# Renmusxd/IsingMonteCarlo

Hardware: AMD Instinct MI355X
Metric: spin-op updates/sec (whole node), 32×32 TFIM, 1024 replicas at 1/2/4/8 GPUs (higher is better)
Workload: dtype u32 op words, f64 acceptance arithmetic

## Files before the change

isingmontecarlo_amd/csrc/sse_cluster.hip.h:

```cpp
#pragma once
#include "sse_cluster_pass.hip.h"

namespace sse {

#define SSE_CLW 16
#define SSE_CL_MAX_VARS 4095u
#define SSE_CLE_TWO (1u << 28)
#define SSE_CLE_LONG (1u << 29)
#define SSE_CLE_CUT (1u << 31)
#define SSE_CL_TOUCHED (1u << 24)

typedef __attribute__((address_space(3))) uint32_t sse_lds_u32;
typedef __attribute__((address_space(3))) uint16_t sse_lds_u16;
typedef __attribute__((address_space(3))) uint8_t sse_lds_u8;
#define LDS32B(a) (*(sse_lds_u32 *)(uintptr_t)(a))
#define LDS16B(a) (*(sse_lds_u16 *)(uintptr_t)(a))
#define LDS8B(a) (*(sse_lds_u8 *)(uintptr_t)(a))
__device__ __forceinline__ void lds_cas32(uint32_t addr, uint32_t expect, uint32_t val) {
    (void)__hip_atomic_compare_exchange_strong((sse_lds_u32 *)(uintptr_t)addr, &expect, val, __ATOMIC_RELAXED, __ATOMIC_RELAXED, __HIP_MEMORY_SCOPE_WORKGROUP);
}

__device__ __forceinline__ uint32_t lds_ld16(uint32_t addr) {
    uint32_t v = LDS16B(addr);
    asm("" : "+v"(v));
    return v;
}
#define SSE_CL_MISC_DUMMY 12u

struct ClLds {
    uint32_t o_tab;
    uint32_t o_state;
    uint32_t o_touch;
    uint32_t o_misc;
    uint32_t o_chn;
    uint32_t o_chtr;
    uint32_t o_ent;
    uint32_t o_frozen, o_froot;
    uint32_t o_parent;
    uint32_t end;
    __host__ __device__ __forceinline__ void carve(uint32_t N, uint32_t nwords, uint32_t Nb, uint32_t ufcap, bool has_long) {
        uint32_t base = 0;
        o_tab = base; base += Nb + 1u;
        o_state = base; base += nwords;
        o_touch = base; base += nwords;
        o_misc = base; base += 16u;
        o_chn = base; base += SSE_MAX_CHUNKS;
        o_chtr = base; base += SSE_MAX_CHUNKS;
        o_ent = base; base += (uint32_t)SSE_CLW * (N + 1u);
        o_frozen = base; base += has_long ? (ufcap + 31u) / 32u : 0u;
        o_froot = base; base += has_long ? (ufcap + 31u) / 32u : 0u;
        o_parent = base;
        end = base + (ufcap + 1u) / 2u;
    }
};
static inline __host__ __device__ bool cl_ids_fit(uint32_t N, uint32_t S, uint32_t ufcap) {
    return S < ufcap && S < 65535u && ((size_t)S + 31) / 32 <= (size_t)SSE_CLW * (N + 1);
}
static inline __host__ __device__ uint32_t cl_list_cap(uint32_t N, uint32_t S) {
    const size_t tab = (size_t)SSE_CLW * (N + 1), bits = ((size_t)S + 31) / 32;
    return bits < tab ? (uint32_t)(2 * (tab - bits)) : 0u;
}

extern "C" __device__ int sse_cl_llvm_writelane(int, int, int) __asm("llvm.amdgcn.writelane.i32");
__device__ __forceinline__ uint32_t cl_writelane(uint32_t v, uint32_t x, int l) { return (uint32_t)sse_cl_llvm_writelane((int)x, l, (int)v); }

__device__ __forceinline__ uint32_t cl_union_wave(const UFA<false> &uf, uint32_t a, uint32_t b) {
    for (;;) {
        uint32_t xa = a, xb = b, pa = uf.get(a), pb = uf.get(b);
        while ((pa != xa) | (pb != xb)) { xa = pa; xb = pb; pa = uf.get(xa); pb = uf.get(xb); }
        if (a != xa) uf.set(a, xa);
        if (b != xb) uf.set(b, xb);
        if (xa == xb) return xa;
        const uint32_t lo = min(xa, xb), hi = max(xa, xb);
        uf.set(hi, lo);
        SSE_WAVE_FENCE();
        if (uf.get(hi) == lo) return lo;
        a = xa; b = xb;
    }
}

#ifndef SSE_CL_FIND_LEVELS
#define SSE_CL_FIND_LEVELS 4
#endif
template <int K, bool HAS_LONG, int PHASE>
__global__ __launch_bounds__(SSE_CLW * 64, 4) void cluster_kernel(DevBatch B, SweepArgs A) {
    constexpr int W = SSE_CLW, NT = W * 64;
    constexpr uint32_t TS = 64u * K;
    static_assert(K == 2 || K == 4, "ids are stored two rows per dword");
    ClLds L;
    L.carve(B.N, B.nwords, B.Nb, B.lds_ufcap, HAS_LONG);
    const int tid = threadIdx.x, lane = tid & 63, wave = __builtin_amdgcn_readfirstlane(tid >> 6);
    const uint32_t r = blockIdx.x;
    const uint32_t N = B.N, nwords = B.nwords;
    const int n = (int)B.n[r];
    const uint32_t C = B.ntrans[r], M = B.cutoff[r], err = B.err[r];
    if (err) return;
    const uint32_t S = N + C + (uint32_t)(W - 1) * N;
    if (n == 0 || C == 0u || !cl_ids_fit(N, S, B.lds_ufcap)) {
        if (tid == 0) B.aux[r] = 1u;
        return;
    }
    UFA<false> uf;
    uf.gparent = nullptr; uf.gfrozen = nullptr; uf.gfroot = nullptr;
    uf.o_parent = L.o_parent; uf.o_frozen = L.o_frozen; uf.o_froot = L.o_froot;
    uint64_t epoch = B.epoch[r];
    uint32_t *ops = B.ops + (size_t)r * B.stride;
    uint32_t *ids = B.segs + (size_t)r * B.stride;
    const bool DEFER = A.defer_flips != 0u && B.flipb != nullptr;
// ... 169 lines not shown
    SSE_STAMP(1);

    for (uint32_t v = tid; v < N; v += NT) {
        uint32_t t = 0;
#pragma unroll 4
        for (uint32_t w2 = 0; w2 < (uint32_t)W; ++w2) {
            const uint32_t x = LDSW(L.o_ent, w2 * (N + 1u) + v);
            t |= x;
            const uint32_t seg_end = x & 0xFFFFu;
            const uint32_t nxt = (w2 + 1u == (uint32_t)W) ? v : N + C + w2 * N + v;
            if (seg_end != nxt) uf_union(uf, seg_end, nxt);
        }
        if (t >> 24) atomicOr(&LDSW(L.o_touch, v >> 5), 1u << (v & 31));
    }
    __syncthreads();
    SSE_STAMP(2);
    const uint32_t o_bits = L.o_ent, o_list = L.o_ent + (S + 31u) / 32u;
    const uint32_t list_cap = cl_list_cap(N, S);
    uint32_t myclusters = 0;
    for (uint32_t i0 = 0; i0 < S; i0 += NT) {
        const uint32_t i = i0 + tid;
        const bool inr = i < S;
        bool isroot = false;
        if (inr) {
            const uint32_t root = uf_find_ro(uf, i);
            uf.set(i, root);
            if constexpr (HAS_LONG)
                if ((uf.frozen_get(i >> 5) >> (i & 31)) & 1u) { uf.froot_or(root >> 5, 1u << (root & 31)); LDSW(L.o_misc, MISC_ANYFROZEN) = 1u; }
            isroot = root == i;
            if (isroot & (i < N + C)) {
                const bool touched = (i >= N) || ((LDSW(L.o_touch, i >> 5) >> (i & 31)) & 1u);
                if (touched) myclusters++;
            }
        }
        const uint64_t m = sse_ballot(isroot);
        if (m) {
            uint32_t base = 0;
            if (lane == 0) base = atomicAdd(&LDSW(L.o_misc, MISC_LOOP_A), (uint32_t)popc64(m));
            base = (uint32_t)__builtin_amdgcn_readfirstlane((int)base);
            const uint32_t pos = base + popc64(m & lanemask_lt(lane));
            if (isroot && pos < list_cap) LDSH(o_list, pos) = (uint16_t)i;
        }
    }
    for (uint32_t i = tid; i < (S + 31u) / 32u; i += NT) LDSW(o_bits, i) = 0u;
    __syncthreads();
    SSE_STAMP(3);
    const Rng rng = make_rng(B, r, epoch);
    const uint32_t nroots = LDSW(L.o_misc, MISC_LOOP_A);
    if (nroots <= list_cap) {
        for (uint32_t k = tid; k < nroots; k += NT) {
            const uint32_t root = LDSH(o_list, k);
            const uint4 o = rng.draw(SSE_TAG_CLUSTER, root);
            const uint32_t isfrozen = HAS_LONG ? (uf.froot_get(root >> 5) >> (root & 31)) & 1u : 0u;
            if (!isfrozen && u01(o.x) < A.prob) atomicOr(&LDSW(o_bits, root >> 5), 1u << (root & 31));
        }
        __syncthreads();
        for (uint32_t i = tid; i < S; i += NT) {
            const uint32_t root = uf.get(i);
            uf.set(i, (LDSW(o_bits, root >> 5) >> (root & 31)) & 1u);
        }
    } else {
        for (uint32_t i = tid; i < S; i += NT) {
            const uint32_t root = uf.get(i);
            const uint4 o = rng.draw(SSE_TAG_CLUSTER, root);
            const uint32_t isfrozen = HAS_LONG ? (uf.froot_get(root >> 5) >> (root & 31)) & 1u : 0u;
            uf.set(i, (!isfrozen && u01(o.x) < A.prob) ? 1u : 0u);
        }
    }
    if (tid == 0) uf.set(S, 0u);
    {
        uint32_t c = myclusters;
        for (int off = 32; off > 0; off >>= 1) c += __shfl_down(c, off);
        if (lane == 0 && c) atomicAdd(&LDSW(L.o_misc, MISC_NCLUST), c);
    }
    __syncthreads();
    SSE_STAMP(4);

    if (DEFER) {
        uint32_t cutnext = N + cutbase;
        uint8_t *fb = B.flipb + (size_t)r * B.stride;
        constexpr int D = 3;
        const uint32_t *mskw = reinterpret_cast<const uint32_t *>(msk);
        uint32_t qid[D][K / 2], qmk[D], bpend[K];
        auto issue = [&](int slot, uint32_t pt) {
            const uint32_t pc = pt < pend ? pt : pbeg;
#pragma unroll
            for (int j = 0; j < K; j += 2) qid[slot][j / 2] = row_ld(ids, (pc >> 1) + (uint32_t)(j * 32 + lane));
            qmk[slot] = row_ld(mskw, (pc >> 6) * 4u + (uint32_t)(lane & 15));
        };
#pragma unroll
        for (int d = 0; d < D; ++d) issue(d, pbeg + (uint32_t)d * TS);
#pragma unroll
        for (int j = 0; j < K; ++j) bpend[j] = 0u;
        uint32_t pprev = pbeg;
        bool first = true;
        for (uint32_t p0 = pbeg; p0 < pend; p0 += TS) {
            uint32_t id2[K / 2];
#pragma unroll
            for (int j = 0; j < K / 2; ++j) id2[j] = qid[0][j];
            const uint32_t mkv = qmk[0];
#pragma unroll
            for (int d = 0; d + 1 < D; ++d) {
#pragma unroll
                for (int j = 0; j < K / 2; ++j) qid[d][j] = qid[d + 1][j];
                qmk[d] = qmk[d + 1];
            }
            if (!first) {
#pragma unroll
                for (int j = 0; j < K; ++j) fb[pprev + (uint32_t)(j * 64 + lane)] = (uint8_t)bpend[j];
            }
            first = false;
            pprev = p0;
            issue(D - 1, p0 + (uint32_t)D * TS);
#pragma unroll
            for (int j = 0; j < K; ++j) {
                const uint64_t cutm = (uint64_t)(uint32_t)__builtin_amdgcn_readlane((int)mkv, 4 * j) | ((uint64_t)(uint32_t)__builtin_amdgcn_readlane((int)mkv, 4 * j + 1) << 32);
                const uint32_t own = __builtin_amdgcn_mbcnt_hi((uint32_t)(cutm >> 32), __builtin_amdgcn_mbcnt_lo((uint32_t)cutm, cutnext));
                const uint32_t idin = (j & 1) ? (id2[j / 2] >> 16) : (id2[j / 2] & 0xFFFFu);
                const uint32_t f1 = LDS16B(par_b + 2u * idin), f2 = LDS16B(par_b + 2u * own);
                uint32_t m_other = (0u - f1) & 0xFu;
                if constexpr (HAS_LONG) {
                    const uint64_t twom = (uint64_t)(uint32_t)__builtin_amdgcn_readlane((int)mkv, 4 * j + 2) | ((uint64_t)(uint32_t)__builtin_amdgcn_readlane((int)mkv, 4 * j + 3) << 32);
                    m_other &= sel64(twom, vgpr_copy_u32(0xFu), vgpr_copy_u32(0x5u));
                }
                bpend[j] = sel64(cutm, f1 | (f2 << 2), m_other);
                cutnext += (uint32_t)popc64(cutm);
            }
        }
        if (pbeg < pend) {
#pragma unroll
            for (int j = 0; j < K; ++j) fb[pprev + (uint32_t)(j * 64 + lane)] = (uint8_t)bpend[j];
        }
    } else
    {
        uint32_t cutnext = N + cutbase;
        const uint32_t E1 = B.E + 1u;
        uint32_t wnext[K], inext[K / 2], wpend[K];
#pragma unroll
        for (int j = 0; j < K; ++j) { wnext[j] = row_ld(ops, pbeg + (uint32_t)(j * 64 + lane)); wpend[j] = wnext[j]; }
#pragma unroll
        for (int j = 0; j < K; j += 2) inext[j / 2] = row_ld(ids, (pbeg >> 1) + (uint32_t)(j * 32 + lane));
        uint32_t pprev = pbeg;
        for (uint32_t p0 = pbeg; p0 < pend; p0 += TS) {
            uint32_t word[K], id2[K / 2];
#pragma unroll
            for (int j = 0; j < K; ++j) word[j] = wnext[j];
#pragma unroll
            for (int j = 0; j < K / 2; ++j) id2[j] = inext[j];
            {
#pragma unroll
                for (int j = 0; j < K; ++j) row_st(ops, pprev + (uint32_t)(j * 64 + lane), wpend[j]);
                pprev = p0;
                const uint32_t pn0 = p0 + TS < pend ? p0 + TS : p0;
#pragma unroll
                for (int j = 0; j < K; ++j) wnext[j] = row_ld(ops, pn0 + (uint32_t)(j * 64 + lane));
#pragma unroll
                for (int j = 0; j < K; j += 2) inext[j / 2] = row_ld(ids, (pn0 >> 1) + (uint32_t)(j * 32 + lane));
            }
            uint32_t f1[K], f2[K];
            uint64_t cutm[K];
#pragma unroll
            for (int j = 0; j < K; ++j) {
                cutm[j] = sse_ballot(((word[j] >> 4) - E1) < N);
                const uint32_t own = __builtin_amdgcn_mbcnt_hi((uint32_t)(cutm[j] >> 32), __builtin_amdgcn_mbcnt_lo((uint32_t)cutm[j], cutnext));
                const uint32_t idin = (j & 1) ? (id2[j / 2] >> 16) : (id2[j / 2] & 0xFFFFu);
                f1[j] = LDS16B(par_b + 2u * idin);
                f2[j] = LDS16B(par_b + 2u * own);
                cutnext += (uint32_t)popc64(cutm[j]);
            }
#pragma unroll
            for (int j = 0; j < K; ++j) {
                const uint32_t allbits = (((word[j] >> 4) - 1u) < B.E) ? 0xFu : 0x5u;
                const uint32_t m_other = (0u - f1[j]) & allbits;
                const uint32_t m_cut = f1[j] | (f2[j] << 2);
                wpend[j] = word[j] ^ sel64(cutm[j], m_cut, m_other);
            }
        }
        if (pbeg < pend) {
#pragma unroll
            for (int j = 0; j < K; ++j) row_st(ops, pprev + (uint32_t)(j * 64 + lane), wpend[j]);
        }
    }
    for (uint32_t v0 = (uint32_t)wave * 64u; v0 < N; v0 += NT) {
        const uint32_t v = v0 + (uint32_t)lane;
        const uint64_t fm = sse_ballot(v < N && (uf.get(v) & 1u) != 0u);
        const uint32_t i = (v0 >> 5) + (uint32_t)lane;
        if (lane < 2 && i < nwords) LDSW(L.o_state, i) ^= (lane ? (uint32_t)(fm >> 32) : (uint32_t)fm) & LDSW(L.o_touch, i);
    }
    __syncthreads();
    SSE_STAMP(5);
    const uint32_t nclusters = LDSW(L.o_misc, MISC_NCLUST);
    epoch++;
    uint64_t a0 = 0, a1 = 0, a2 = 0, a3 = 0, a6 = 0;
    if (A.domask & SSE_DO_FREE) {
        const Rng rngf = make_rng(B, r, epoch);
        for (uint32_t v0 = (uint32_t)wave * 64u; v0 < N; v0 += NT) {
            const uint32_t v = v0 + (uint32_t)lane;
            const bool isfree = v < N && !((LDSW(L.o_touch, v >> 5) >> (v & 31u)) & 1u);
            uint32_t bit = 0u;
            if (isfree) bit = rngf.draw(SSE_TAG_FREE, v).x >> 31;
            const uint64_t fm = sse_ballot(isfree), bm = sse_ballot(bit != 0u);
            const uint32_t i = (v0 >> 5) + (uint32_t)lane;
            if (fm != 0ull && lane < 2 && i < nwords) {
                const uint32_t f = lane ? (uint32_t)(fm >> 32) : (uint32_t)fm, b = lane ? (uint32_t)(bm >> 32) : (uint32_t)bm;
                LDSW(L.o_state, i) = (LDSW(L.o_state, i) & ~f) | b;
            }
        }
        __syncthreads();
        epoch++;
    }
    if (A.sampling_freq && (A.step0 + 1) % A.sampling_freq == 0) {
        if (tid == 0) LDSW(L.o_misc, MISC_LOOP_A) = 0u;
        __syncthreads();
        uint32_t up = 0;
// ... 19 lines not shown
```

isingmontecarlo_amd/csrc/sse_core.hip.h:

```cpp
#pragma once
#include <hip/hip_runtime.h>
#include <stdint.h>
#include "../../include/sse_format.h"
#include "sse_batch.h"

namespace sse {

#ifdef SSE_PHASE_TIMING
#define SSE_STAMP(slot) do { if (threadIdx.x == 0) { const unsigned long long t_ = __builtin_amdgcn_s_memrealtime(); B.dbg[(size_t)r * 16 + (slot)] += t_ - dbg_t0; dbg_t0 = t_; } } while (0)
#define SSE_STAMP_INIT unsigned long long dbg_t0 = __builtin_amdgcn_s_memrealtime()
#else
#define SSE_STAMP(slot) do { } while (0)
#define SSE_STAMP_INIT do { } while (0)
#endif

__device__ __forceinline__ uint32_t philox_bump(uint32_t k, uint32_t w) {
    uint32_t r;
    const uint32_t ks = (uint32_t)__builtin_amdgcn_readfirstlane((int)k);
    asm volatile("s_add_u32 %0, %1, %2" : "=s"(r) : "s"(ks), "s"(w) : "scc");
    return r;
}
__device__ __forceinline__ uint4 philox4x32_10(uint32_t c0, uint32_t c1, uint32_t c2, uint32_t c3, uint32_t k0,
                                               uint32_t k1) {
#pragma unroll
    for (int i = 0; i < 10; ++i) {
        const uint64_t p0 = (uint64_t)0xD2511F53u * (uint64_t)c0, p1 = (uint64_t)0xCD9E8D57u * (uint64_t)c2;
        const uint32_t hi0 = (uint32_t)(p0 >> 32), lo0 = (uint32_t)p0, hi1 = (uint32_t)(p1 >> 32), lo1 = (uint32_t)p1;
        uint32_t n0 = __builtin_amdgcn_bitop3_b32(hi1, c1, k0, 0x96), n2 = __builtin_amdgcn_bitop3_b32(hi0, c3, k1, 0x96);
        c0 = n0; c1 = lo1; c2 = n2; c3 = lo0;
        if (i < 9) { k0 = philox_bump(k0, 0x9E3779B9u); k1 = philox_bump(k1, 0xBB67AE85u); }
    }
    return make_uint4(c0, c1, c2, c3);
}

struct Rng {
    uint32_t k0, k1, replica, epoch_lo, epoch_hi24;
#ifdef SSE_PHASE_TIMING
    uint32_t dbgx;
#endif
    __device__ __forceinline__ uint4 draw(uint32_t tag, uint32_t index) const {
#ifdef SSE_PHASE_TIMING
        if (dbgx & 2u) {
            const uint32_t h = (index * 0x9E3779B9u) ^ (epoch_lo * 0x85EBCA6Bu) ^ (replica * 0xC2B2AE35u) ^ tag;
            return make_uint4(h * 0x27D4EB2Fu, h ^ (h >> 15), h * 0x165667B1u, h ^ (h << 13));
        }
#endif
        return philox4x32_10(index, epoch_lo, replica, (tag << 24) | epoch_hi24, k0, k1);
    }
};
__device__ __forceinline__ Rng make_rng(const DevBatch &B, uint32_t r, uint64_t epoch) {
    Rng g;
    g.k0 = B.seed_lo; g.k1 = B.seed_hi; g.replica = B.rid ? B.rid[r] : B.replica_offset + r;
    g.epoch_lo = (uint32_t)epoch; g.epoch_hi24 = (uint32_t)(epoch >> 32) & 0xFFFFFFu;
#ifdef SSE_PHASE_TIMING
    g.dbgx = B.dbg_flags;
#endif
    return g;
}
__device__ __forceinline__ double u01(uint32_t x) { return (double)x * (1.0 / 4294967296.0); }

struct Bd {
    uint32_t a, c, kp;
    double w;
};
__device__ __forceinline__ uint32_t bd_kind(const Bd &b) { return b.kp & SSE_BOND_KIND_MASK; }

__device__ __forceinline__ double bond_weight(const Bd &b, uint32_t in, uint32_t out) {
    const uint32_t kind = b.kp & SSE_BOND_KIND_MASK, pref = (b.kp >> 2) & 1u;
    const uint32_t aligned = ((in ^ (in >> 1)) & 1u) ^ 1u;
    const uint32_t sat = (kind == SSE_BOND_TWO_SITE) ? (uint32_t)(aligned == pref) : (uint32_t)((in & 1u) == pref);
    const bool ok = (kind == SSE_BOND_TRANSVERSE) | ((in == out) & (sat != 0u));
    return ok ? b.w : 0.0;
}

__device__ __forceinline__ double op_weight(const DevBatch &B, uint32_t b, const Bd &d, uint32_t in, uint32_t out) {
    if (B.mats) return B.mats[(size_t)b * 16u + (in | (out << 2))];
    return bond_weight(d, in, out);
}

extern __shared__ __align__(16) uint32_t lds_raw[];
#define LDSW(off, i) lds_raw[(off) + (i)]
#define LDSI(off, i) (reinterpret_cast<int &>(lds_raw[(off) + (i)]))
#define LDSH(off, i) (reinterpret_cast<uint16_t *>(lds_raw)[2u * (off) + (i)])
#define LDSB(off, i) (reinterpret_cast<uint8_t *>(lds_raw)[4u * (off) + (i)])
#ifdef SSE_PHASE_TIMING
#define SSE_DBG(B, bit) (((B).dbg_flags & (bit)) != 0u)
#else
#define SSE_DBG(B, bit) false
#endif
#define SSE_WAVE_FENCE() __builtin_amdgcn_fence(__ATOMIC_ACQ_REL, "wavefront")

template <int W>
struct Lds {
    uint32_t o_state;
    uint32_t o_touch;
    uint32_t o_touch8;
    uint32_t o_tot;
    uint32_t o_chg;
    uint32_t o_misc;
    uint32_t o_chn;
    uint32_t o_chtr;
    uint32_t o_edges;
    uint32_t o_signs;
    uint32_t o_cur;
    uint32_t o_cl;
    uint32_t o_frozen;
    uint32_t o_froot;
    uint32_t o_parent;
    uint32_t end;
    uint32_t end_diag;
    __host__ __device__ __forceinline__ void carve(uint32_t N, uint32_t nwords, uint32_t ufcap, uint32_t ledges, uint32_t has_long, bool tg = false,
                                                   uint32_t pm_words = 0, bool diag_only = false) {
        uint32_t base = 0;
        o_state = base; base += nwords;
        o_touch = base; base += nwords;
        if (tg) N = 0;
        o_touch8 = base; base += diag_only ? 0u : (N + 3) / 4;
        o_tot = base; base += 2 * W;
        o_chg = base; base += 2 * W;
        o_misc = base; base += 16;
        o_chn = base; base += SSE_MAX_CHUNKS;
        o_chtr = base; base += SSE_MAX_CHUNKS;
        o_edges = base; base += ledges;
        o_signs = base; base += pm_words;
        o_cur = base; base += diag_only ? (W * N + 3) / 4 : (W * N + 1) / 2;
        end_diag = o_cur + (W * N + 3) / 4;
        o_cl = base; base += diag_only ? 0u : (W * N + 3) / 4;
        o_frozen = base; base += has_long ? (ufcap + 31) / 32 : 0u;
        o_froot = base; base += has_long ? (ufcap + 31) / 32 : 0u;
        o_parent = base;
// ... 135 lines not shown
```

isingmontecarlo_amd/csrc/sse_fast.hip.h:

```cpp
#pragma once
#include "sse_accept.h"
#include "sse_loop.hip.h"

namespace sse {

#define SSE_FAST_MAX_VARS 4096u
#define LDS8(a) (reinterpret_cast<uint8_t *>(lds_raw)[(a)])
#define SSE_FAST_CLASS_J 0u
#define SSE_FAST_CLASS_G 1u
#define SSE_FAST_CLASS_H 2u

__device__ __forceinline__ uint32_t bfi32(uint32_t mask, uint32_t a, uint32_t b) {
    uint32_t r;
    asm("v_bfi_b32 %0, %1, %2, %3" : "=v"(r) : "v"(mask), "v"(a), "v"(b));
    return r;
}

struct FastLds {
    uint32_t o_nb;
    uint32_t o_xch;
    uint32_t o_tab;
    uint32_t o_spin;
    uint32_t o_dummy;
    uint32_t end;
};
template <int W>
__host__ __device__ __forceinline__ FastLds fast_carve(const Lds<W> &L, const DevBatch &B) {
    FastLds F;
    static_assert(4 * W >= 3 + 8, "o_xch: eight words behind an alignment gap of up to three, inside o_tot + o_chg");
    uint32_t base = (L.o_edges + 3u) & ~3u;
    F.o_nb = base; base += 16;
    F.o_xch = (L.o_tot + 3u) & ~3u;
    F.o_tab = base; base += B.Nb;
    F.o_spin = base; base += B.N;
    F.o_dummy = base; base += 64;
    F.end = base;
    return F;
}

__device__ __forceinline__ uint32_t fast_entry(const DevBatch &B, uint32_t b, uint32_t ce) {
    if (b < B.E) {
        const uint32_t a = ce & SSE_CE_VAR_MASK, c = (ce >> 15) & SSE_CE_VAR_MASK, pref = (ce >> 30) & 1u;
        return a | (c << 12) | ((pref ? 0x9u : 0x6u) << 24) | (3u << 28) | (SSE_FAST_CLASS_J << 30);
    }
    const uint32_t s1 = b - B.E;
    if (s1 < B.N) return s1 | (s1 << 12) | (0xFu << 24) | (1u << 28) | (SSE_FAST_CLASS_G << 30);
    const uint32_t v = s1 - B.N;
    return v | (v << 12) | ((B.hpos ? 0x8u : 0x1u) << 24) | (1u << 28) | (SSE_FAST_CLASS_H << 30);
}

template <int K, bool F64>
__device__ __forceinline__ void diagonal_fast(const DevBatch &B, const Lds<4> &L, const FastLds &F, uint32_t r, const Rng &rng, double beta,
                                              uint32_t M, int &n_io, int &ntrans_io, uint32_t &gr, uint32_t fbmask) {
    constexpr int W = 4, NT = W * 64;
    constexpr uint32_t TS = (uint32_t)(NT * K);
    static_assert(K == 2 || K == 4, "rows p and p + 64 share one Philox call");
    const int tid = threadIdx.x, lane = tid & 63, wave = __builtin_amdgcn_readfirstlane(tid >> 6);
    uint32_t *ops = B.ops + (size_t)r * B.stride;
    const uint8_t *flipb = (fbmask ? B.flipb : reinterpret_cast<const uint8_t *>(B.ops)) + (size_t)r * B.stride;
    auto ld_word = [&](uint32_t idx) -> uint32_t {
        return row_ld(ops, idx) ^ ((uint32_t)*reinterpret_cast<const uint8_t *>(reinterpret_cast<const char *>(flipb) + (size_t)idx) & fbmask);
    };
    const uint32_t N = B.N, Nb = B.Nb, E = B.E;
    for (uint32_t i = tid; i < N; i += NT) LDSW(F.o_spin, i) = ((LDSW(L.o_state, i >> 5) >> (i & 31)) & 1u) * 0x01010101u;
    __syncthreads();

    const uint32_t ntiles = (M + TS - 1) / TS;
    int n_start = n_io, ntrans = 0;
    const uint32_t m_later = (uint32_t)((0x0101010100ull << (8 * wave)) & 0xFFFFFFFFull);
    const uint32_t m_earlier = 0x01010101u & ((1u << (8 * wave)) - 1u);
    const uint32_t spin_my = 4u * F.o_spin + (uint32_t)wave;
    const uint32_t markhi = (127u - (uint32_t)lane) << 1;

    const uint32_t dummy_b = 4u * (F.o_dummy + (uint32_t)lane);
    auto evmask32 = [](uint32_t wd) -> uint32_t { return 0u - ((wd ^ (wd >> 2)) & 1u); };
    const uint32_t spin_b = 4u * (F.o_spin - 1u - E);
    auto decode = [&](uint32_t wd) -> uint32_t { return bfi32(evmask32(wd), spin_b + 4u * (wd >> 4), dummy_b); };
    auto propagate = [&](const uint32_t (&vb)[K], uint32_t mask) {
        if (mask == 0u) return;
#pragma unroll
        for (int j = 0; j < K; ++j) atomicXor(reinterpret_cast<uint32_t *>(reinterpret_cast<char *>(lds_raw) + vb[j]), mask);
    };

    uint32_t wnext[K], vnext[K];
#pragma unroll
    for (int j = 0; j < K; ++j) { wnext[j] = ld_word((uint32_t)(wave * 64 * K + j * 64 + lane)); vnext[j] = decode(wnext[j]); }
    propagate(vnext, m_later);
    __syncthreads();
    const uint32_t lane2 = 2u * (uint32_t)lane;
    const uint32_t vM = vgpr_copy_u32(M), vM1 = vgpr_copy_u32(M + 1u), vzero = vgpr_copy_u32(0u);
    const uint32_t vnever_hi = vgpr_copy_u32((uint32_t)(SSE_ACCEPT_NEVER_INSERT >> 32)), vnever_thr = vgpr_copy_u32((uint32_t)SSE_ACCEPT_NEVER_REMOVE);
    uint32_t ch = (uint32_t)(wave * 64 * K) / B.CH, chpos = (uint32_t)(wave * 64 * K) % B.CH;

    for (uint32_t tile = 0; tile < ntiles; ++tile) {
#if SSE_ROTATE_PRIO
        if ((tile & (SSE_ROTATE_PRIO - 1u)) == 0u) sse_set_prio((tile / SSE_ROTATE_PRIO) + blockIdx.x);
#endif
        uint32_t word[K], vcur[K];
#pragma unroll
        for (int j = 0; j < K; ++j) { word[j] = wnext[j]; vcur[j] = vnext[j]; }
        const uint32_t pbase = tile * TS + (uint32_t)(wave * 64 * K + lane);
        {
            const uint32_t pn = (tile + 1 < ntiles ? pbase + TS : pbase);
#pragma unroll
            for (int j = 0; j < K; ++j) wnext[j] = ld_word(pn + (uint32_t)(j * 64));
        }
        const bool partial = tile * TS + TS > M;

        uint32_t cbv[K], neww[K], ent[K], bnd[K], rr1[K];
        uint64_t acci[K], accr[K];
        uint32_t chi[K];
        uint32_t clo[K];
        int32_t thr[K];
        double un[K], nb[K];
        uint64_t insm[K], remm[K];
        {
            uint4 rnd = make_uint4(0, 0, 0, 0);
#pragma unroll
            for (int j = 0; j < K; ++j) {
                const uint32_t wd = word[j];
                if ((j & 1) == 0) rnd = rng.draw(SSE_TAG_DIAG, pbase + (uint32_t)(j * 64));
                const uint32_t r0 = (j & 1) ? rnd.z : rnd.x;
                rr1[j] = (j & 1) ? rnd.w : rnd.y;
                const uint64_t occm = sse_ballot(wd != 0u);
                bnd[j] = sel64(occm, (wd >> 4) - 1u, __umulhi(r0, Nb));
                ent[j] = LDSW(F.o_tab, bnd[j]);
            }
        }
        uint32_t sub0[K];
#pragma unroll
        for (int j = 0; j < K; ++j) {
            const uint32_t e = ent[j], inb = word[j] & 1u;
            const uint32_t va = e & 0xFFFu, vc = (e >> 12) & 0xFFFu;
            const uint32_t adr_a = spin_my + 4u * va, adr_c = spin_my + 4u * vc;
            const uint32_t mark = markhi | inb;
            const uint32_t adr_w = vcur[j] + (uint32_t)wave;
            const uint64_t evm = sse_ballot(vcur[j] != dummy_b);
            LDS8(adr_w) = (uint8_t)mark;
            SSE_WAVE_FENCE();
            const uint32_t ea = LDS8(adr_a), ec = LDS8(adr_c);
            uint32_t sa, sc;
            const uint64_t dup = sse_ballot(ea != mark) & evm;
            if (!dup) {
                sa = (ea ^ ((ea + lane2) >> 8)) & 1u;
                sc = (ec ^ ((ec + lane2) >> 8)) & 1u;
                SSE_WAVE_FENCE();
                LDS8(adr_w) = (uint8_t)(inb ^ 1u);
            } else {
                sa = ea & 1u; sc = ec & 1u;
                bool seen_a = false, seen_c = false;
                uint64_t m = evm;
                while (m) {
                    const int Ls = __ffsll((long long)m) - 1;
                    m &= m - 1;
                    const bool later = lane > Ls;
                    const uint32_t vL = __builtin_amdgcn_readlane(va, Ls), inL = __builtin_amdgcn_readlane(inb, Ls);
                    if (va == vL) { sa = later ? (inL ^ 1u) : (seen_a ? sa : inL); seen_a = true; }
                    if (vc == vL) { sc = later ? (inL ^ 1u) : (seen_c ? sc : inL); seen_c = true; }
                    if (lane == Ls) LDS8(adr_a) = (uint8_t)(inL ^ 1u);
                }
                SSE_WAVE_FENCE();
            }
            sub0[j] = sa | (sc << 1);
        }
#pragma unroll
        for (int j = 0; j < K; ++j) {
            const uint32_t e = ent[j], wd = word[j];
            const uint32_t okbit = (e >> (24u + sub0[j])) & 1u;
            const uint32_t sub = sub0[j] & (e >> 28) & 3u;
            const uint4 cls = *reinterpret_cast<const uint4 *>(&lds_raw[F.o_nb + 4u * (e >> 30)]);
            const double num_lo = __hiloint2double((int)cls.w, (int)cls.z);
            uint64_t im = sse_ballot(okbit > wd);
            if (partial) im &= sse_ballot(pbase + (uint32_t)(j * 64) < M);
            const uint64_t rm = sse_ballot(wd != 0u) & ~sse_ballot(vcur[j] != dummy_b);
            if constexpr (F64) {
                un[j] = (double)rr1[j] * num_lo;
                nb[j] = __hiloint2double((int)cls.y, (int)cls.x);
                insm[j] = im; remm[j] = rm;
            } else {
                clo[j] = cls.x;
                chi[j] = sel64(im, cls.y, vnever_hi);
                thr[j] = (int32_t)sel64(rm, (uint32_t)sse_accept_remove_threshold(rr1[j], num_lo), vnever_thr);
            }
            cbv[j] = sel64(im, vM, vM1);
            neww[j] = sel64(im, ((bnd[j] + 1u) << 4) | sub | (sub << 2), vzero);
            acci[j] = 0ull; accr[j] = 0ull;
        }

        int npref[K];
#pragma unroll
        for (int j = 0; j < K; ++j) npref[j] = n_start;
        int tot_all = 0, base = 0, wtot = 0;
        bool first = true;
        for (;;) {
            wtot = 0;
            uint64_t diff = 0ull;
#pragma unroll
            for (int j = 0; j < K; ++j) {
                const int t = (int)(cbv[j] - (uint32_t)npref[j]);
                uint64_t ai, ar;
                if constexpr (F64) {
                    const double td = (double)t;
                    ai = sse_ballot((double)rr1[j] * td < nb[j]) & insm[j];
                    ar = sse_ballot(un[j] < td) & remm[j];
                } else {
                    ai = sse_ballot(sse_accept_insert(rr1[j], (uint32_t)t, ((uint64_t)chi[j] << 32) | clo[j]));
                    ar = sse_ballot(sse_accept_remove(t, thr[j]));
                }
                diff |= (ai ^ acci[j]) | (ar ^ accr[j]);
                acci[j] = ai; accr[j] = ar;
                wtot += popc64(ai) - popc64(ar);
            }
            const bool changed = first | (diff != 0ull);
            const uint32_t xch = F.o_xch + 4u * (gr & 1u);
            if (lane == 0) LDSW(xch, wave) = ((uint32_t)wtot << 1) | (changed ? 1u : 0u);
            __syncthreads();
            if (first) {
                propagate(vcur, m_earlier);
#pragma unroll
                for (int j = 0; j < K; ++j) vnext[j] = decode(wnext[j]);
                if (tile + 1 < ntiles) propagate(vnext, m_later);
            }
            const uint4 xw = *reinterpret_cast<const uint4 *>(&lds_raw[xch]);
            const int x4[W] = {__builtin_amdgcn_readfirstlane((int)xw.x), __builtin_amdgcn_readfirstlane((int)xw.y),
                               __builtin_amdgcn_readfirstlane((int)xw.z), __builtin_amdgcn_readfirstlane((int)xw.w)};
            base = 0; tot_all = 0;
#pragma unroll
            for (int w2 = 0; w2 < W; ++w2) {
                const int t = x4[w2] >> 1;
                if (w2 < wave) base += t;
                tot_all += t;
            }
            const uint32_t anychg = (uint32_t)(x4[0] | x4[1] | x4[2] | x4[3]) & 1u;
            gr++;
            if (!first && !anychg) break;
            first = false;
            int run = n_start + base;
#pragma unroll
            for (int j = 0; j < K; ++j) {
                const uint64_t im = acci[j], rm = accr[j];
                const int ci = (int)__builtin_amdgcn_mbcnt_hi((uint32_t)(im >> 32), __builtin_amdgcn_mbcnt_lo((uint32_t)im, (uint32_t)run));
                const int cr = (int)__builtin_amdgcn_mbcnt_hi((uint32_t)(rm >> 32), __builtin_amdgcn_mbcnt_lo((uint32_t)rm, 0u));
                npref[j] = ci - cr;
                run += popc64(im) - popc64(rm);
            }
        }
        const int dn = wtot;
        int dtr = 0;
#pragma unroll
        for (int j = 0; j < K; ++j) {
            const uint32_t fw = sel64(acci[j] | accr[j], neww[j], word[j]);
            row_st(ops, pbase + (uint32_t)(j * 64), fw);
            const uint64_t trm = sse_ballot((ent[j] >> 30) == SSE_FAST_CLASS_G);
            dtr += popc64(acci[j] & trm) - popc64(accr[j] & trm);
        }
        ntrans += dtr;
        if (lane == 0 && (dtr | dn)) {
            if (dn) atomicAdd(&LDSW(L.o_chn, ch), (uint32_t)dn);
            if (dtr) atomicAdd(&LDSW(L.o_chtr, ch), (uint32_t)dtr);
        }
        n_start += tot_all;
        chpos += TS;
        while (chpos >= B.CH) { chpos -= B.CH; ch++; }
    }
    __syncthreads();
    if (lane == 0) LDSI(L.o_tot, wave) = ntrans;
    __syncthreads();
    int dt = 0;
#pragma unroll
    for (int w2 = 0; w2 < W; ++w2) dt += LDSI(L.o_tot, w2);
    __syncthreads();
    ntrans_io += dt;
    n_io = n_start;
}

template <int K, int PHASE, bool F64>
__global__ __launch_bounds__(256, 4) void sweep_fast_kernel(DevBatch B, SweepArgs A) {
    constexpr int W = 4, NT = W * 64;
    Lds<W> L;
    L.carve(B.N, B.nwords, B.lds_ufcap, B.E, B.has_long);
    const FastLds F = fast_carve<W>(L, B);
    const int tid = threadIdx.x;
    const uint32_t r = blockIdx.x;
#ifdef SSE_WG_TIMELINE
    if (tid == 0 && (B.dbg_flags & 32u)) { B.dbg[(size_t)r * 16 + 0] = __builtin_amdgcn_s_memrealtime(); B.dbg[(size_t)r * 16 + 2] = __builtin_amdgcn_s_getreg((4 << 0) | (0 << 6) | (31 << 11)); B.dbg[(size_t)r * 16 + 3] = __builtin_amdgcn_s_getreg((20 << 0) | (0 << 6) | (31 << 11)); }
#endif
    const double beta = A.beta ? A.beta[r] : 0.0;
    for (uint32_t i = tid; i < B.nwords; i += NT) LDSW(L.o_state, i) = B.state[(size_t)r * B.nwords + i];
    for (uint32_t i = tid; i < B.Nb; i += NT) LDSW(F.o_tab, i) = fast_entry(B, i, i < B.E ? B.edges_compact[i] : 0u);
    for (uint32_t i = tid; i < 2 * SSE_MAX_CHUNKS; i += NT) LDSW(L.o_chn, i) = B.chunks[(size_t)r * 2 * SSE_MAX_CHUNKS + i];
    if (tid < 4) {
        const double beta_nb = beta * (double)B.Nb;
        const double w = tid == 0 ? B.wJ : (tid == 1 ? B.gamma : (tid == 2 ? B.wh : 0.0));
        const double num = beta_nb * w;
        if constexpr (F64) *reinterpret_cast<double *>(&lds_raw[F.o_nb + 4u * (uint32_t)tid]) = num * 4294967296.0;
        else *reinterpret_cast<uint64_t *>(&lds_raw[F.o_nb + 4u * (uint32_t)tid]) = sse_accept_insert_const(num);
        *reinterpret_cast<double *>(&lds_raw[F.o_nb + 4u * (uint32_t)tid + 2u]) = num * (1.0 / 4294967296.0);
    }
    __syncthreads();
    int n = (int)B.n[r], ntrans = (int)B.ntrans[r];
    uint32_t M = B.cutoff[r], err = B.err[r], gr = 0, last_out = 0;
    uint64_t epoch = B.epoch[r];
    uint64_t a4 = 0, a5 = 0;
    const uint32_t fbmask = (A.defer_flips && B.flipb && (A.domask & SSE_DO_DIAG) && !err && B.pend[r]) ? 0xFFu : 0u;
    for (uint64_t step = 0; step < A.nsteps; ++step) {
        if (err) break;
        if (A.domask & SSE_DO_DIAG) {
            const Rng rng = make_rng(B, r, epoch);
            diagonal_fast<K, F64>(B, L, F, r, rng, beta, M, n, ntrans, gr, step == 0 ? fbmask : 0u);
            epoch++;
            a5 += M;
            if (A.domask & SSE_DO_GROW) {
                const uint32_t want = (uint32_t)n + (uint32_t)n / 2u;
                if (want > M) { if (want > B.cap) { err = SSE_ERR_CAPACITY; break; } M = want; }
            }
        }
        if (A.domask & SSE_DO_LOOP) {
            __syncthreads();
            for (uint32_t i = tid; i < B.E; i += NT) LDSW(L.o_edges, i) = B.edges_compact[i];
            __syncthreads();
            const Rng rng = make_rng(B, r, epoch);
            last_out = loop_pass<W, true>(B, L, r, rng, M, n, gr, err);
            epoch++;
            a4 += last_out;
            if (err) break;
        }
    }
// ... 17 lines not shown
```

Baseline: 175.2 billion.

## Micro-optimize cluster flip pass, interleave dual Philox draws, simplify diagonal acceptance counters

New measurement: 179.7 billion, median of 6. +2.6%, better.

```diff
diff --git a/isingmontecarlo_amd/csrc/sse_cluster.hip.h b/isingmontecarlo_amd/csrc/sse_cluster.hip.h
--- a/isingmontecarlo_amd/csrc/sse_cluster.hip.h
+++ b/isingmontecarlo_amd/csrc/sse_cluster.hip.h
@@ -24,6 +24,11 @@
     uint32_t v = LDS16B(addr);
     asm("" : "+v"(v));
     return v;
+}
+__device__ __forceinline__ uint32_t cl_low16(uint32_t x) {
+    uint32_t r;
+    asm("v_and_b32 %0, 0xffff, %1" : "=v"(r) : "v"(x));
+    return r;
 }
 #define SSE_CL_MISC_DUMMY 12u
 
@@ -359,43 +364,31 @@
         constexpr int D = 3;
         const uint32_t *mskw = reinterpret_cast<const uint32_t *>(msk);
         uint32_t qid[D][K / 2], qmk[D], bpend[K];
+        const uint32_t lane4 = 4u * (uint32_t)lane, lane15_4 = 4u * (uint32_t)(lane & 15);
         auto issue = [&](int slot, uint32_t pt) {
             const uint32_t pc = pt < pend ? pt : pbeg;
-#pragma unroll
-            for (int j = 0; j < K; j += 2) qid[slot][j / 2] = row_ld(ids, (pc >> 1) + (uint32_t)(j * 32 + lane));
-            qmk[slot] = row_ld(mskw, (pc >> 6) * 4u + (uint32_t)(lane & 15));
+            const char *idt = reinterpret_cast<const char *>(ids + (pc >> 1));
+            const char *mkt = reinterpret_cast<const char *>(mskw + (pc >> 6) * 4u);
+#pragma unroll
+            for (int j = 0; j < K; j += 2)
+                qid[slot][j / 2] = *reinterpret_cast<const uint32_t *>(idt + (size_t)lane4 + (size_t)(j * 128));
+            qmk[slot] = *reinterpret_cast<const uint32_t *>(mkt + (size_t)lane15_4);
         };
-#pragma unroll
-        for (int d = 0; d < D; ++d) issue(d, pbeg + (uint32_t)d * TS);
-#pragma unroll
-        for (int j = 0; j < K; ++j) bpend[j] = 0u;
-        uint32_t pprev = pbeg;
-        bool first = true;
-        for (uint32_t p0 = pbeg; p0 < pend; p0 += TS) {
-            uint32_t id2[K / 2];
-#pragma unroll
-            for (int j = 0; j < K / 2; ++j) id2[j] = qid[0][j];
-            const uint32_t mkv = qmk[0];
-#pragma unroll
-            for (int d = 0; d + 1 < D; ++d) {
-#pragma unroll
-                for (int j = 0; j < K / 2; ++j) qid[d][j] = qid[d + 1][j];
-                qmk[d] = qmk[d + 1];
-            }
-            if (!first) {
-#pragma unroll
-                for (int j = 0; j < K; ++j) fb[pprev + (uint32_t)(j * 64 + lane)] = (uint8_t)bpend[j];
-            }
-            first = false;
-            pprev = p0;
-            issue(D - 1, p0 + (uint32_t)D * TS);
+        auto store = [&](uint32_t pt) {
+            uint8_t *fbt = fb + pt;
+#pragma unroll
+            for (int j = 0; j < K; ++j) fbt[(size_t)(uint32_t)lane + (size_t)(j * 64)] = (uint8_t)bpend[j];
+        };
+        auto tile = [&](int slot) {
+            const uint32_t mkv = qmk[slot];
 #pragma unroll
             for (int j = 0; j < K; ++j) {
                 const uint64_t cutm = (uint64_t)(uint32_t)__builtin_amdgcn_readlane((int)mkv, 4 * j) | ((uint64_t)(uint32_t)__builtin_amdgcn_readlane((int)mkv, 4 * j + 1) << 32);
-                const uint32_t own = __builtin_amdgcn_mbcnt_hi((uint32_t)(cutm >> 32), __builtin_amdgcn_mbcnt_lo((uint32_t)cutm, cutnext));
-                const uint32_t idin = (j & 1) ? (id2[j / 2] >> 16) : (id2[j / 2] & 0xFFFFu);
-                const uint32_t f1 = LDS16B(par_b + 2u * idin), f2 = LDS16B(par_b + 2u * own);
-                uint32_t m_other = (0u - f1) & 0xFu;
+                const uint32_t below = __builtin_amdgcn_mbcnt_hi((uint32_t)(cutm >> 32), __builtin_amdgcn_mbcnt_lo((uint32_t)cutm, 0u));
+                const uint32_t idw = qid[slot][j / 2];
+                const uint32_t idin = (j & 1) ? (idw >> 16) : cl_low16(idw);
+                const uint32_t f1 = LDS16B(par_b + 2u * idin), f2 = LDS16B(par_b + 2u * (cutnext + below));
+                uint32_t m_other = __umul24(f1, 0xFu);
                 if constexpr (HAS_LONG) {
                     const uint64_t twom = (uint64_t)(uint32_t)__builtin_amdgcn_readlane((int)mkv, 4 * j + 2) | ((uint64_t)(uint32_t)__builtin_amdgcn_readlane((int)mkv, 4 * j + 3) << 32);
                     m_other &= sel64(twom, vgpr_copy_u32(0xFu), vgpr_copy_u32(0x5u));
@@ -403,10 +396,24 @@
                 bpend[j] = sel64(cutm, f1 | (f2 << 2), m_other);
                 cutnext += (uint32_t)popc64(cutm);
             }
-        }
+        };
+#pragma unroll
+        for (int d = 0; d < D; ++d) issue(d, pbeg + (uint32_t)d * TS);
         if (pbeg < pend) {
-#pragma unroll
-            for (int j = 0; j < K; ++j) fb[pprev + (uint32_t)(j * 64 + lane)] = (uint8_t)bpend[j];
+            uint32_t p0 = pbeg;
+            for (;;) {
+                bool done = false;
+#pragma unroll
+                for (int d = 0; d < D; ++d) {
+                    if (d > 0 || p0 != pbeg) store(p0 - TS);
+                    tile(d);
+                    issue(d, p0 + (uint32_t)D * TS);
+                    p0 += TS;
+                    if (p0 >= pend) { done = true; break; }
+                }
+                if (done) break;
+            }
+            store(p0 - TS);
         }
     } else
     {
diff --git a/isingmontecarlo_amd/csrc/sse_core.hip.h b/isingmontecarlo_amd/csrc/sse_core.hip.h
--- a/isingmontecarlo_amd/csrc/sse_core.hip.h
+++ b/isingmontecarlo_amd/csrc/sse_core.hip.h
@@ -32,6 +32,21 @@
     }
     return make_uint4(c0, c1, c2, c3);
 }
+__device__ __forceinline__ void philox4x32_10_x2(uint32_t c0a, uint32_t c0b, uint32_t c1, uint32_t c2, uint32_t c3, uint32_t k0, uint32_t k1,
+                                                 uint4 &oa, uint4 &ob) {
+    uint32_t a0 = c0a, a1 = c1, a2 = c2, a3 = c3, b0 = c0b, b1 = c1, b2 = c2, b3 = c3;
+#pragma unroll
+    for (int i = 0; i < 10; ++i) {
+        const uint64_t pa0 = (uint64_t)0xD2511F53u * (uint64_t)a0, pa1 = (uint64_t)0xCD9E8D57u * (uint64_t)a2;
+        const uint64_t pb0 = (uint64_t)0xD2511F53u * (uint64_t)b0, pb1 = (uint64_t)0xCD9E8D57u * (uint64_t)b2;
+        const uint32_t na0 = __builtin_amdgcn_bitop3_b32((uint32_t)(pa1 >> 32), a1, k0, 0x96), na2 = __builtin_amdgcn_bitop3_b32((uint32_t)(pa0 >> 32), a3, k1, 0x96);
+        const uint32_t nb0 = __builtin_amdgcn_bitop3_b32((uint32_t)(pb1 >> 32), b1, k0, 0x96), nb2 = __builtin_amdgcn_bitop3_b32((uint32_t)(pb0 >> 32), b3, k1, 0x96);
+        a0 = na0; a1 = (uint32_t)pa1; a2 = na2; a3 = (uint32_t)pa0;
+        b0 = nb0; b1 = (uint32_t)pb1; b2 = nb2; b3 = (uint32_t)pb0;
+        if (i < 9) { k0 = philox_bump(k0, 0x9E3779B9u); k1 = philox_bump(k1, 0xBB67AE85u); }
+    }
+    oa = make_uint4(a0, a1, a2, a3); ob = make_uint4(b0, b1, b2, b3);
+}
 
 struct Rng {
     uint32_t k0, k1, replica, epoch_lo, epoch_hi24;
@@ -46,6 +61,12 @@
         }
 #endif
         return philox4x32_10(index, epoch_lo, replica, (tag << 24) | epoch_hi24, k0, k1);
+    }
+    __device__ __forceinline__ void draw2(uint32_t tag, uint32_t ia, uint32_t ib, uint4 &oa, uint4 &ob) const {
+#ifdef SSE_PHASE_TIMING
+        if (dbgx & 2u) { oa = draw(tag, ia); ob = draw(tag, ib); return; }
+#endif
+        philox4x32_10_x2(ia, ib, epoch_lo, replica, (tag << 24) | epoch_hi24, k0, k1, oa, ob);
     }
 };
 __device__ __forceinline__ Rng make_rng(const DevBatch &B, uint32_t r, uint64_t epoch) {
diff --git a/isingmontecarlo_amd/csrc/sse_fast.hip.h b/isingmontecarlo_amd/csrc/sse_fast.hip.h
--- a/isingmontecarlo_amd/csrc/sse_fast.hip.h
+++ b/isingmontecarlo_amd/csrc/sse_fast.hip.h
@@ -88,7 +88,7 @@
     propagate(vnext, m_later);
     __syncthreads();
     const uint32_t lane2 = 2u * (uint32_t)lane;
-    const uint32_t vM = vgpr_copy_u32(M), vM1 = vgpr_copy_u32(M + 1u), vzero = vgpr_copy_u32(0u);
+    const uint32_t vzero = vgpr_copy_u32(0u);
     const uint32_t vnever_hi = vgpr_copy_u32((uint32_t)(SSE_ACCEPT_NEVER_INSERT >> 32)), vnever_thr = vgpr_copy_u32((uint32_t)SSE_ACCEPT_NEVER_REMOVE);
     uint32_t ch = (uint32_t)(wave * 64 * K) / B.CH, chpos = (uint32_t)(wave * 64 * K) % B.CH;
 
@@ -107,7 +107,7 @@
         }
         const bool partial = tile * TS + TS > M;
 
-        uint32_t cbv[K], neww[K], ent[K], bnd[K], rr1[K];
+        uint32_t neww[K], ent[K], bnd[K], rr1[K];
         uint64_t acci[K], accr[K];
         uint32_t chi[K];
         uint32_t clo[K];
@@ -115,11 +115,13 @@
         double un[K], nb[K];
         uint64_t insm[K], remm[K];
         {
-            uint4 rnd = make_uint4(0, 0, 0, 0);
+            uint4 rnds[K / 2];
+            if constexpr (K == 4) rng.draw2(SSE_TAG_DIAG, pbase, pbase + 128u, rnds[0], rnds[1]);
+            else rnds[0] = rng.draw(SSE_TAG_DIAG, pbase);
 #pragma unroll
             for (int j = 0; j < K; ++j) {
                 const uint32_t wd = word[j];
-                if ((j & 1) == 0) rnd = rng.draw(SSE_TAG_DIAG, pbase + (uint32_t)(j * 64));
+                const uint4 rnd = rnds[j / 2];
                 const uint32_t r0 = (j & 1) ? rnd.z : rnd.x;
                 rr1[j] = (j & 1) ? rnd.w : rnd.y;
                 const uint64_t occm = sse_ballot(wd != 0u);
@@ -172,7 +174,7 @@
             const double num_lo = __hiloint2double((int)cls.w, (int)cls.z);
             uint64_t im = sse_ballot(okbit > wd);
             if (partial) im &= sse_ballot(pbase + (uint32_t)(j * 64) < M);
-            const uint64_t rm = sse_ballot(wd != 0u) & ~sse_ballot(vcur[j] != dummy_b);
+            const uint64_t rm = sse_ballot(wd != 0u) & sse_ballot(vcur[j] >= dummy_b);
             if constexpr (F64) {
                 un[j] = (double)rr1[j] * num_lo;
                 nb[j] = __hiloint2double((int)cls.y, (int)cls.x);
@@ -182,14 +184,13 @@
                 chi[j] = sel64(im, cls.y, vnever_hi);
                 thr[j] = (int32_t)sel64(rm, (uint32_t)sse_accept_remove_threshold(rr1[j], num_lo), vnever_thr);
             }
-            cbv[j] = sel64(im, vM, vM1);
-            neww[j] = sel64(im, ((bnd[j] + 1u) << 4) | sub | (sub << 2), vzero);
+            neww[j] = sel64(im, __umul24(sub, 5u) + ((bnd[j] << 4) + 16u), vzero);
             acci[j] = 0ull; accr[j] = 0ull;
         }
 
-        int npref[K];
-#pragma unroll
-        for (int j = 0; j < K; ++j) npref[j] = n_start;
+        uint32_t q[K];
+#pragma unroll
+        for (int j = 0; j < K; ++j) q[j] = M - (uint32_t)n_start;
         int tot_all = 0, base = 0, wtot = 0;
         bool first = true;
         for (;;) {
@@ -197,15 +198,14 @@
             uint64_t diff = 0ull;
 #pragma unroll
             for (int j = 0; j < K; ++j) {
-                const int t = (int)(cbv[j] - (uint32_t)npref[j]);
+                const int t = (int)q[j];
                 uint64_t ai, ar;
                 if constexpr (F64) {
-                    const double td = (double)t;
-                    ai = sse_ballot((double)rr1[j] * td < nb[j]) & insm[j];
-                    ar = sse_ballot(un[j] < td) & remm[j];
+                    ai = sse_ballot((double)rr1[j] * (double)t < nb[j]) & insm[j];
+                    ar = sse_ballot(un[j] < (double)(t + 1)) & remm[j];
                 } else {
                     ai = sse_ballot(sse_accept_insert(rr1[j], (uint32_t)t, ((uint64_t)chi[j] << 32) | clo[j]));
-                    ar = sse_ballot(sse_accept_remove(t, thr[j]));
+                    ar = sse_ballot(sse_accept_remove(t + 1, thr[j]));
                 }
                 diff |= (ai ^ acci[j]) | (ar ^ accr[j]);
                 acci[j] = ai; accr[j] = ar;
@@ -235,14 +235,13 @@
             gr++;
             if (!first && !anychg) break;
             first = false;
-            int run = n_start + base;
+            uint32_t mrun = M - (uint32_t)(n_start + base);
 #pragma unroll
             for (int j = 0; j < K; ++j) {
                 const uint64_t im = acci[j], rm = accr[j];
-                const int ci = (int)__builtin_amdgcn_mbcnt_hi((uint32_t)(im >> 32), __builtin_amdgcn_mbcnt_lo((uint32_t)im, (uint32_t)run));
-                const int cr = (int)__builtin_amdgcn_mbcnt_hi((uint32_t)(rm >> 32), __builtin_amdgcn_mbcnt_lo((uint32_t)rm, 0u));
-                npref[j] = ci - cr;
-                run += popc64(im) - popc64(rm);
+                const uint32_t ci = __builtin_amdgcn_mbcnt_hi((uint32_t)(im >> 32), __builtin_amdgcn_mbcnt_lo((uint32_t)im, 0u));
+                q[j] = __builtin_amdgcn_mbcnt_hi((uint32_t)(rm >> 32), __builtin_amdgcn_mbcnt_lo((uint32_t)rm, mrun - ci));
+                mrun -= (uint32_t)(popc64(im) - popc64(rm));
             }
         }
         const int dn = wtot;
```
